# NilanEkanayake/TiTok-Video

Measured on AMD Instinct MI355X. Metric: video clips/sec encode+decode (whole node), higher is better.
Workload: dtype bf16

## Files before the change

### titok_video_amd/csrc/ttv_api.hip

```cpp
#include <stdarg.h>
#include <stdio.h>
#include <stdlib.h>
#include <string.h>

#include "ttv_common.h"
#include "ttv_kernels.h"

static thread_local char g_err[512] = "";

void ttv_set_error(const char* fmt, ...) {
  va_list ap;
  va_start(ap, fmt);
  vsnprintf(g_err, sizeof(g_err), fmt, ap);
  va_end(ap);
}

int g_ttv_prof_class = 0;
bool ttv_sw_enc_latent_last() { static const bool v = ttv_env_flag("TTV_ENC_LATENT_LAST", true); return v; }
bool ttv_enc_latent_rows_only(const ttv_tower_dims* d, const ttv_batch* b) {
  return ttv_sw_enc_latent_last() && !(g_ttv_debug & TTV_DBG_ENC_ALL_ROWS) && d->kind == TTV_ENCODER && b->latent_rows && b->sum_tokens > 0 &&
         b->sum_tokens < b->total_rows;
}
bool ttv_sw_keel_f32sum() { static const bool v = ttv_env_flag("TTV_KEEL_F32SUM", false); return v; }
bool ttv_sw_fused_patch() { static const bool v = ttv_env_flag("TTV_FUSED_PATCH", true); return v; }
// ... 527 lines not shown
  return ttvk_mlp_fused(ao, ldao, attn_post_gain, attn_alpha, x, ldx, mlp_packed, inner, y, ldy, ffd_post_gain, ffd_alpha, eps, M,
                        next ? &nx : nullptr, (hipStream_t)stream);
}

int ttv_fill_const_rows(void* x, int dtype, int ld, const int32_t* rows_map, int rows, int width, const float* mask_token,
                        const float* gain, float eps, void* stream) {
  TTV_CHECK_ARG(rows == 0 || (x && rows_map && mask_token && gain), "fill_const_rows: null buffer");
  return ttvk_fill_const_rows(x, dtype, ld, rows_map, rows, width, mask_token, gain, eps, (hipStream_t)stream);
}

int ttv_decoder_embed(const void* codes, int token_size, const void* w, const void* bias, const float* mask_token, const float* gain,
                      void* x, int dtype, int ld, const int32_t* rows_map, int rows, int width, float eps, void* stream) {
  TTV_CHECK_ARG(rows == 0 || (codes && w && bias && mask_token && gain && x && rows_map), "decoder_embed: null buffer");
  return ttvk_dec_embed(codes, token_size, w, bias, mask_token, gain, x, dtype, ld, rows_map, rows, width, eps, (hipStream_t)stream);
}

int ttv_attention(const void* qkvg, int ld, void* out, int ldo, const int32_t* cu_seqlens, const int32_t* qblocks, int n_qblocks,
                  int q_heads, int kv_heads, int head_dim, int flags, int dtype, void* stream) {
  TTV_CHECK_ARG(n_qblocks == 0 || (qkvg && out && cu_seqlens && qblocks), "attention: null buffer");
  return ttvk_attention(qkvg, ld, out, ldo, cu_seqlens, qblocks, n_qblocks, q_heads, kv_heads, head_dim, flags, dtype, (hipStream_t)stream);
}
int ttv_attention64(const void* qkvg, int ld, void* out, int ldo, const int32_t* cu_seqlens, const int32_t* items, int n_items, int q_heads,
                    int kv_heads, int head_dim, int flags, int dtype, void* stream) {
  TTV_CHECK_ARG(dtype == TTV_BF16 && head_dim == 64, "attention64: bf16, head_dim 64 only");
  return ttvk_attention64(qkvg, ld, out, ldo, cu_seqlens, items, n_items, q_heads, kv_heads, flags, (hipStream_t)stream);
}

int ttv_rmsnorm_mx(const void* in, int in_dtype, int ld_in, void* out, int out_dtype, int ld_out, const float* gain, int rows, int width,
                   float eps, float* next_rstd, void* mx_q, void* mx_s, void* stream) {
  TTV_CHECK_ARG(rows >= 0 && (rows == 0 || (in && out && gain)), "rmsnorm_mx: null buffer");
  TTV_CHECK_ARG(!mx_q == !mx_s, "rmsnorm_mx: the image needs both its element and its scale buffer");
  return ttvk_rmsnorm(in, in_dtype, ld_in, nullptr, out, out_dtype, ld_out, nullptr, gain, rows, width, eps, (hipStream_t)stream, next_rstd, mx_q, mx_s);
}

int ttv_attention_mxout(const void* qkvg, int ld, void* out_q, void* out_mx, int ld_mx, const int32_t* cu_seqlens, const int32_t* qblocks,
                        int n_qblocks, int q_heads, int kv_heads, void* stream) {
  TTV_CHECK_ARG(n_qblocks >= 0 && (n_qblocks == 0 || (qkvg && out_q && out_mx && cu_seqlens && qblocks)), "attention_mxout: null buffer");
  return ttvk_attention_mxout(qkvg, ld, out_q, out_mx, ld_mx, cu_seqlens, qblocks, n_qblocks, q_heads, kv_heads, (hipStream_t)stream);
}

int ttv_linear_fp8_mx_geglu_q(const void* xq, int ldx, const void* x_mx, const float* x_row_scale, const void* wq, int ldw, const void* w_mx,
                              const float* w_row_scale, void* hq, void* hq_mx, int M, int N, int K, void* stream) {
  TTV_CHECK_ARG(M == 0 || (xq && wq && x_mx && w_mx && hq && hq_mx), "linear_fp8_mx_geglu_q: null buffer");
  GemmArgs a = gemm_args(TTV_BF16, xq, ldx, wq, ldw, M, N, K, hq, N);
  a.yq = hq; a.yq_mx = hq_mx;
  return ttvk_gemm_fp8(EPI_GEGLU, a, x_row_scale, w_row_scale, (hipStream_t)stream, x_mx, w_mx);
}

int ttv_row_rstd(const void* x, int dtype, int ldx, float* rstd, int rows, int width, float eps, void* stream) {
  TTV_CHECK_ARG(rows >= 0 && (rows == 0 || (x && rstd)), "row_rstd: null buffer");
  TTV_CHECK_ARG(ldx >= width, "row_rstd: leading dim smaller than the width");
  return ttvk_row_rstd(x, dtype, ldx, rstd, rows, width, eps, (hipStream_t)stream);
}

int ttv_linear_rowscale(const void* x, int ldx, const void* w, int ldw, const float* row_scale, int epilogue, const float* rope_cs, int d_model,
                        int gqa_dim, void* y, int ldy, int M, int N, int K, int dtype, void* stream) {
  TTV_CHECK_ARG(M == 0 || (x && w && y), "linear_rowscale: null buffer");
  TTV_CHECK_ARG(epilogue >= 0 && epilogue <= 2, "linear_rowscale: epilogue 0 (store), 1 (qkv + rotary) or 2 (GEGLU)");
  GemmArgs a = gemm_args(dtype, x, ldx, w, ldw, M, N, K, y, ldy);
  if (epilogue == 1) {
    TTV_CHECK_ARG(rope_cs && N == 2 * d_model + 2 * gqa_dim && K == d_model, "linear_rowscale: qkv epilogue needs rope_cs, N = 2 d_model + 2 gqa_dim and K = d_model");
    a = gemm_rope_qk(a, rope_cs, d_model, gqa_dim);
  }
  a.row_scale = row_scale;
  return ttvk_gemm(epilogue == 0 ? EPI_STORE : epilogue == 1 ? EPI_QKV_ROPE : EPI_GEGLU, a, (hipStream_t)stream);
}

int ttv_patch_gather(const void* const* clips, const int32_t* clip_desc, int clip0, int n_clips, int patch_t, int patch_h, int patch_w,
                     int channels, void* patches, int ld, int dtype, int max_patches_per_clip, void* stream) {
  TTV_CHECK_ARG(n_clips == 0 || (clips && clip_desc && patches), "patch_gather: null buffer");
  return ttvk_patch_copy(false, (void* const*)clips, clip_desc, clip0, n_clips, patch_t, patch_h, patch_w, channels, patches, ld, dtype, max_patches_per_clip, (hipStream_t)stream);
}

int ttv_patch_embed_norm(const void* const* clips, const int32_t* clip_desc, const int32_t* patch_rows, const int32_t* row_seq, int n_clips,
                         int patch_t, int patch_h, int patch_w, int channels, const void* w, int ldw, const void* bias, const float* mask_token,
                         const float* gain, float eps, void* x, int ldx, int rows, int width, int dtype, void* stream) {
  TTV_CHECK_ARG(rows == 0 || (clips && clip_desc && patch_rows && row_seq && w && bias && mask_token && gain && x), "patch_embed_norm: null buffer");
  const int pd = channels * patch_t * patch_h * patch_w;
  if (!ttvk_patch_embed_norm_supported(dtype, width, pd, patch_w)) {
    ttv_set_error("patch_embed_norm: only bf16, width 256, patch_w 8 and a patch vector that is a multiple of 64");
    return TTV_ERR_UNSUPPORTED;
  }
  return ttvk_patch_embed_norm((void* const*)clips, 0, n_clips, clip_desc, patch_rows, row_seq, patch_t, patch_h, patch_w, pd, w, ldw, bias,
                               mask_token, gain, eps, x, ldx, rows, (hipStream_t)stream);
}

int ttv_patch_scatter(const void* patches, int ld, const int32_t* clip_desc, int clip0, int n_clips, int patch_t, int patch_h, int patch_w,
                      int channels, void* const* clips, int dtype, int max_patches_per_clip, void* stream) {
  TTV_CHECK_ARG(n_clips == 0 || (clips && clip_desc && patches), "patch_scatter: null buffer");
  return ttvk_patch_copy(true, clips, clip_desc, clip0, n_clips, patch_t, patch_h, patch_w, channels, (void*)patches, ld, dtype, max_patches_per_clip, (hipStream_t)stream);
}

int64_t ttv_tower_workspace_bytes(const ttv_tower_dims* dims, const ttv_batch* batch) {
  if (check_dims(dims, batch) != TTV_OK) return -1;
  return carve(dims, batch, nullptr).total;
}

int ttv_encoder_forward(const ttv_tower_dims* d, const ttv_tower_weights* w, const ttv_batch* b, const void* const* clips,
                        const ttv_fsq_params* fsq, float* z, void* codes, int32_t* indices, float* bounded, void* workspace,
                        int64_t workspace_bytes, void* stream) {
  TTV_TRY(check_dims(d, b));
  TTV_CHECK_ARG(d->kind == TTV_ENCODER, "encoder_forward: dims.kind is not TTV_ENCODER");
  TTV_CHECK_ARG(w && w->layers && clips && workspace, "encoder_forward: null argument");
  TTV_CHECK_ARG(fsq || z, "encoder_forward: neither fsq nor z requested");
  TTV_CHECK_ARG(!fsq || (codes && indices), "encoder_forward: fsq needs codes and indices buffers");
  hipStream_t s = (hipStream_t)stream;
  TowerWs ws = carve(d, b, (char*)workspace);
  TTV_CHECK_ARG(ws.total <= workspace_bytes, "encoder_forward: workspace too small (%lld < %lld)", (long long)workspace_bytes, (long long)ws.total);
  const int dm = d->width, dt = d->dtype, P = b->sum_patches, pd = patch_dim(d);

  static const bool embed_env = ttv_env_flag("TTV_PATCH_EMBED_FUSED", true);
  if (embed_env && !(g_ttv_debug & TTV_DBG_PATCH_EMBED_UNFUSED) && fused_patch_ok(d, b, dt) && w->proj_in_b && w->mask_token &&
      ttvk_patch_embed_norm_supported(dt, dm, pd, d->patch_w)) {
    TTV_TRY(ttvk_patch_embed_norm((void* const*)clips, 0, b->n_clips, b->clip_desc, b->patch_rows, b->row_seq, d->patch_t, d->patch_h, d->patch_w,
                                  pd, w->proj_in_w, pd, w->proj_in_b, w->mask_token, w->ln_pre_p, d->eps, ws.x, dm, P, s));
  } else {
    const bool gather = fused_patch_ok(d, b, dt) && pd != 256;
    if (!gather) TTV_TRY(patch_copy_all(false, (void* const*)clips, d, b, ws.pa, dt, s));
    GemmArgs a = gemm_args(dt, ws.pa, pd, w->proj_in_w, pd, P, dm, pd, ws.pb, dm);
    a.bias = w->proj_in_b; a.add_scalar = w->mask_token;
    a.split3 = (dt == TTV_F32 && w->f32_split3) ? 1 : 0;
    if (gather) {
      a.gather = 1; a.clips = (void* const*)clips; a.n_clips = b->n_clips; a.clip_desc = b->clip_desc; a.patch_rows = b->patch_rows;
      a.row_seq = b->row_seq; a.patch_t = d->patch_t; a.patch_h = d->patch_h; a.patch_w = d->patch_w;
    }
    TTV_TRY(ttvk_gemm(EPI_STORE, a, s));
    TTV_TRY(ttvk_rmsnorm(ws.pb, dt, dm, nullptr, ws.x, dt, dm, b->patch_rows, w->ln_pre_p, P, dm, d->eps, s));
  }
  TTV_TRY(ttvk_fill_const_rows(ws.x, dt, dm, b->latent_rows, b->sum_tokens, dm, w->mask_token, w->ln_pre_t, d->eps, s));

  TTV_TRY(run_layers(d, w, b, ws, s));

  TTV_TRY(ttvk_enc_tail(ws.x, dt, dm, b->latent_rows, b->sum_tokens, dm, w->ln_post, d->eps, w->proj_out_w, w->proj_out_b, d->token_size, fsq, z, codes, indices, bounded, s));
  return TTV_OK;
}

int64_t ttv_dec_l0_const_bytes(const ttv_tower_dims* d, int patch_rows) {
  if (!d || patch_rows <= 0 || d->dtype != TTV_BF16 || d->width != 256 || d->head_dim != 64 || d->kv_heads <= 0) {
    ttv_set_error("dec_l0_const_bytes: bf16 decoders of width 256 and head_dim 64 only");
    return -1;
  }
  if (patch_rows % 128) {
    ttv_set_error("dec_l0_const_bytes: patch_rows must be a multiple of 128");
    return -1;
  }
  const int64_t nq = 2 * (int64_t)d->width + 2 * (int64_t)d->kv_heads * d->head_dim;
  return align256(patch_rows * nq * 2) + align256(ttvk_attention_swp_state_floats(patch_rows, d->q_heads) * 4 + 4) + align256((int64_t)patch_rows * d->width * 2);
}

int ttv_dec_l0_const_build(const ttv_tower_dims* d, const ttv_tower_weights* w, const int32_t* iota, const float* rope_cs, const int32_t* rope_ids,
                           const float* rope_base, int patch_rows, void* block, int64_t block_bytes, int64_t* state_offset, int64_t* flag_offset,
                           void* stream) {
  TTV_CHECK_ARG(d && w && w->layers && iota && rope_cs && block && patch_rows > 0, "dec_l0_const_build: null argument");
  const int64_t need = ttv_dec_l0_const_bytes(d, patch_rows);
  if (need < 0) return TTV_ERR_UNSUPPORTED;
  TTV_CHECK_ARG(d->kind == TTV_DECODER && need <= block_bytes && (uintptr_t)block % 256 == 0, "dec_l0_const_build: not a decoder, or block too small / unaligned");
  const ttv_layer_weights& lw = w->layers[0];
  if (!lw.to_qkv_pn || !lw.qkv_q_prescaled) {
    ttv_set_error("dec_l0_const_build: layer 0 needs the folded, q-pre-scaled to_qkv weight");
    return TTV_ERR_UNSUPPORTED;
  }
  hipStream_t s = (hipStream_t)stream;
  const int dm = d->width, g = d->kv_heads * d->head_dim, nq = 2 * dm + 2 * g, dt = d->dtype;
  char* const rows = (char*)block;
  const int64_t state_floats = ttvk_attention_swp_state_floats(patch_rows, d->q_heads);
  float* const state = (float*)(rows + align256((int64_t)patch_rows * nq * 2));
  char* const x = (char*)state + align256(state_floats * 4 + 4);
  if (state_offset) *state_offset = (char*)state - rows;
  if (flag_offset) *flag_offset = (char*)(state + state_floats) - rows;
  TTV_TRY(ttvk_fill_const_rows(x, dt, dm, iota, patch_rows, dm, w->mask_token, w->ln_pre_p, d->eps, s));
  GemmArgs a = gemm_rope_qk(gemm_args(dt, x, dm, lw.to_qkv_pn, dm, patch_rows, nq, dm, rows, nq), rope_cs, dm, g);
  a.prenorm = 1; a.eps = d->eps;
  a.rope_ids = rope_ids; a.rope_base = rope_ids ? rope_base : nullptr;
  TTV_TRY(ttvk_gemm(EPI_QKV_ROPE, a, s));
  if (hipMemsetAsync(state + state_floats, 0, 4, s) != hipSuccess) {
    ttv_set_error("dec_l0_const_build: hipMemsetAsync failed");
    return TTV_ERR_LAUNCH;
  }
  return ttvk_attention_swp_dump(rows, nq, patch_rows, d->q_heads, d->kv_heads, state, s);
}

int ttv_decoder_forward(const ttv_tower_dims* d, const ttv_tower_weights* w, const ttv_batch* b, const void* codes,
                        void* const* clips_out, void* workspace, int64_t workspace_bytes, void* stream) {
  return ttv_decoder_forward_const(d, w, b, codes, clips_out, workspace, workspace_bytes, nullptr, stream);
}

int ttv_decoder_forward_const(const ttv_tower_dims* d, const ttv_tower_weights* w, const ttv_batch* b, const void* codes,
                              void* const* clips_out, void* workspace, int64_t workspace_bytes, const ttv_dec_l0_const* l0, void* stream) {
  TTV_TRY(check_dims(d, b));
  TTV_CHECK_ARG(d->kind == TTV_DECODER, "decoder_forward: dims.kind is not TTV_DECODER");
  TTV_CHECK_ARG(w && w->layers && codes && clips_out && workspace, "decoder_forward: null argument");
  hipStream_t s = (hipStream_t)stream;
  TowerWs ws = carve(d, b, (char*)workspace);
  TTV_CHECK_ARG(ws.total <= workspace_bytes, "decoder_forward: workspace too small (%lld < %lld)", (long long)workspace_bytes, (long long)ws.total);
  const int dm = d->width, dt = d->dtype, P = b->sum_patches, pd = patch_dim(d);

  TTV_TRY(ttvk_dec_embed(codes, d->token_size, w->proj_in_w, w->proj_in_b, w->mask_token, w->ln_pre_t, ws.x, dt, dm, b->latent_rows, b->sum_tokens, dm, d->eps, s));
  TTV_TRY(ttvk_fill_const_rows(ws.x, dt, dm, b->patch_rows, P, dm, w->mask_token, w->ln_pre_p, d->eps, s));

  TTV_TRY(run_layers(d, w, b, ws, s, l0));

  GemmArgs a = gemm_args(dt, nullptr, dm, w->proj_out_w, dm, P, pd, dm, ws.pa, pd);
  a.split3 = (dt == TTV_F32 && w->f32_split3) ? 1 : 0;
  a.bias = w->proj_out_b;
  if (dt == TTV_BF16 && dm == 256 && w->proj_out_pn && pd % 8 == 0) {
    a.x = ws.x; a.x_rows = b->patch_rows; a.w = w->proj_out_pn; a.prenorm = 1; a.eps = d->eps;
  } else {
    TTV_TRY(ttvk_rmsnorm(ws.x, dt, dm, b->patch_rows, ws.pb, dt, dm, nullptr, w->ln_post, P, dm, d->eps, s));
    a.x = ws.pb;
  }
  if (fused_patch_ok(d, b, dt) && dm == 256) {
    a.clips = clips_out; a.n_clips = b->n_clips; a.clip_desc = b->clip_desc; a.patch_rows = b->patch_rows; a.row_seq = b->row_seq;
// ... 197 lines not shown
```

### titok_video_amd/csrc/ttv_kernels.h

```cpp
#pragma once
#include <hip/hip_runtime.h>
#include <stdint.h>

#include "../../include/titok_hip.h"

int ttvk_rmsnorm(const void* in, int in_dtype, int ld_in, const int* src_rows, void* out, int out_dtype, int ld_out,
                 const int* dst_rows, const float* gain, int rows, int d, float eps, hipStream_t s, float* next_rstd = nullptr,
                 void* mx_q = nullptr, void* mx_s = nullptr,
                 int split_image = 0);
int ttvk_row_rstd(const void* in, int dtype, int ld_in, float* rstd, int rows, int d, float eps, hipStream_t s);
int ttvk_copy_rows(const void* src, int64_t ld_src_bytes, const int* src_rows, void* dst, int64_t ld_dst_bytes, const int* dst_rows, int rows,
                   int row_bytes, hipStream_t s);
int ttvk_fill_const_rows(void* x, int dtype, int ld, const int* rows_map, int rows, int d, const float* mask_token,
                         const float* gain, float eps, hipStream_t s);
int ttvk_dec_embed(const void* codes, int C, const void* w, const void* bias, const float* mask_token, const float* gain,
                   void* x, int dtype, int ld, const int* rows_map, int rows, int d, float eps, hipStream_t s);
int ttvk_fsq_forward(const ttv_fsq_params* p, const void* z, int z_dtype, int rows, void* codes, int codes_dtype, int* indices,
                     float* bounded, hipStream_t s);
int ttvk_fsq_indices_to_codes(const ttv_fsq_params* p, const int* indices, int rows, void* codes, int codes_dtype, hipStream_t s);
int ttvk_enc_tail(const void* x, int dtype, int ld, const int* rows_map, int rows, int d, const float* gain, float eps,
                  const void* w, const void* bias, int C, const ttv_fsq_params* fsq, float* z_out, void* codes, int* indices,
                  float* bounded, hipStream_t s);
int ttvk_patch_copy(bool scatter, void* const* clips, const int* clip_desc, int clip0, int n_clips, int pt, int ph, int pw,
                    int C, void* patches, int ld, int dtype, int max_patches, hipStream_t s);
int ttvk_rope_apply(void* x, int dtype, int ld, int rows, int heads, const float* cs, hipStream_t s);
int ttvk_histogram(const int* idx, int n, int64_t* counts, int size, hipStream_t s);
int ttvk_quant_rows_fp8(const void* in, int in_dtype, int ld_in, const float* gain, float eps, void* out, int ld_out, float* scales, int rows,
                        int d, hipStream_t s);

int ttvk_split3_pack(const float* w, int ldw, void* out, int ldo, int rows, int K, hipStream_t s);
int64_t ttvk_mx_scale_ld(int d);
int ttvk_quant_mx_fp8(const void* in, int in_dtype, int ld_in, void* out, int ld_out, void* mx, float* row_scales, int rows, int d, hipStream_t s);

int ttvk_clip_from_u8(const void* frames, long long n_pix, void* clip, int dtype, hipStream_t s);

int ttvk_clip_resample_u8(void* const* src, void* const* dst, const int32_t* geom, int n_clips, int dtype, hipStream_t s);

enum GemmEpilogue {
  EPI_STORE = 0,
  EPI_QKV_ROPE,
  EPI_GEGLU,
  EPI_RESID_T,
  EPI_RESID_F32,
  EPI_RESID_NORM,
  EPI_STORE_PATCH,
  EPI_BIAS_PLAIN,
  EPI_BIAS_GELU,
  EPI_BIAS_RESID_F32R,
};

struct GemmArgs {
  const void* x; int ldx;
  const void* w; int ldw;
  int M, N, K;
  void* y; int ldy;
  const void* bias;
  const float* add_scalar;
  const void* resid; int ldr;
  float alpha;
  const float* rope_cs;
  const int* rope_ids; const float* rope_base;
  int rope_q_end, rope_k_begin, rope_k_end;
  int dtype;
  const float* norm_gain;
  float* sum_f32; int ld_sum;
  void* y2; int ldy2; const float* norm_gain2;
  void* yq; void* yq_mx;
  int split3;
  int x_image, y_image;
  int prenorm;
  const float* row_scale;
  const int* x_rows;
  float eps;
  int gather;
  void* const* clips;
  int n_clips;
  const int* clip_desc;
  const int* patch_rows;
  const int* row_seq;
  int patch_t, patch_h, patch_w;
  int resid_rows;
  int tile_run, tile_period;
  int panel_lo;
};
struct ClipPtrs { void* p[TTV_MAX_CLIPS_PER_LAUNCH]; };
int ttvk_gemm(GemmEpilogue epi, const GemmArgs& a, hipStream_t s);
int ttvk_gemm_fp8(GemmEpilogue epi, const GemmArgs& a, const float* x_scale, const float* w_scale, hipStream_t s, const void* x_mx = nullptr,
                  const void* w_mx = nullptr);
bool ttvk_gemm_supports_resid_norm(int dtype, int N, int K);
bool ttvk_gemm_qkv_tiles_supported(int d_model, int gqa_dim, int ldw);

bool ttvk_patch_embed_norm_supported(int dtype, int width, int patch_dim, int patch_w);
int ttvk_patch_embed_norm(void* const* clips, int clip0, int n_clips, const int* clip_desc, const int* patch_rows, const int* row_seq,
                          int patch_t, int patch_h, int patch_w, int patch_dim, const void* w, int ldw, const void* bias,
                          const float* mask_token, const float* gain, float eps, void* x, int ldx, int M, hipStream_t s);

int ttvk_attention(const void* qkvg, int ld, void* out, int ldo, const int* cu_seqlens, const int* qblocks, int n_qblocks,
                   int q_heads, int kv_heads, int head_dim, int flags, int dtype, hipStream_t s, float* lse_out = nullptr,
                   void* out_raw = nullptr);

bool ttvk_attention_takes_swp(int flags);
int ttvk_attention_swp(const void* qkvg, int ld, void* out, int ldo, const int* cu_seqlens, const int* qblocks, int n_qblocks,
                       int q_heads, int kv_heads, int gate_mul, hipStream_t s, const void* rows2 = nullptr, int kwin = 0,
                       const float* state = nullptr);
int64_t ttvk_attention_swp_state_floats(int n_rows, int q_heads);
int ttvk_attention_swp_dump(const void* rows, int ld, int n_rows, int q_heads, int kv_heads, float* state, hipStream_t s);
int ttvk_attention_mxout(const void* qkvg, int ld, void* out_q, void* out_mx, int ld_mx, const int* cu_seqlens, const int* qblocks,
                         int n_qblocks, int q_heads, int kv_heads, hipStream_t s);

int ttvk_attention64(const void* qkvg, int ld, void* out, int ldo, const int* cu_seqlens, const int* items, int n_items, int q_heads,
                     int kv_heads, int flags, hipStream_t s);

int ttvk_vq_norms(const void* cb, int dtype, int ld, int N, int C, float* cnorm, hipStream_t s);
int64_t ttvk_vq_workspace_bytes(int rows);
int ttvk_vq_l2_argmin(const void* z, int dtype, int ldz, const void* cb, int ldc, const float* cnorm, int rows, int N, int C, int* indices,
                      float* best_dist, void* workspace, int64_t workspace_bytes, hipStream_t s);
int ttvk_vq_lookup(const void* cb, int dtype, int ldc, const int* indices, int rows, int C, void* codes, int ldo, hipStream_t s);
int ttvk_vq_lookup_bwd(const void* dcodes, int dtype, int ld, const int* indices, int rows, int C, float* dcb, int ldc, hipStream_t s);

int64_t ttvk_vq_train_workspace_bytes(int rows, int N);
int ttvk_vq_commit_forward(const void* z, int dtype, int ldz, const void* cb, int ldc, const int* idx, int rows, int N, int C, float* loss,
                           void* workspace, int64_t workspace_bytes, hipStream_t s);
int ttvk_vq_commit_backward(const void* g, int ldg, const void* z, int ldz, const void* e, int lde, int dtype, int rows, int C, double scale,
                            void* dz, int ldd, hipStream_t s);
int ttvk_vq_ema_stats(const void* z, int dtype, int ldz, const int* idx, int rows, int N, int C, const float* cluster_size, float dead_threshold,
                      uint64_t seed, const int64_t* ema_step, int rank, int world_size, float* stats, void* workspace, int64_t workspace_bytes,
                      hipStream_t s);
int ttvk_vq_ema_update(const float* stats, float* cluster_size, float* embed_avg, float* codebook, void* copy, int copy_dtype, float* cnorm,
                       int64_t* ema_step, int N, int C, float decay, float one_minus_decay, float eps, float dead_threshold, void* workspace,
                       int64_t workspace_bytes, hipStream_t s);

bool ttvk_mlp_fused_supported(int dtype, int width, int inner);
struct MlpNextQkv {
  void* qkv; int ld;
  const float* rope_cs;
  int rows;
  int rope_q_end, rope_k_begin, rope_k_end;
};
int64_t ttvk_mlp_pack_bytes(int inner, int next_qkv_rows);
int ttvk_mlp_pack(const void* w12_folded, const void* w3, const void* wo, const void* next_qkv_folded, int next_qkv_rows, int inner,
                  void* packed, hipStream_t s);
int ttvk_mlp_fused(const void* ao, int ldao, const float* front_gain, float front_alpha, const void* x, int ldx, const void* packed,
                   int inner, void* y, int ldy, const float* post_gain, float alpha, float eps, int M, const MlpNextQkv* nq, hipStream_t s);

int ttvk_l1_loss(void* const* recon, void* const* target, void* const* grad, const int* sizes, int n_clips, int total_clips, int dtype,
                 float* loss, hipStream_t s);
int ttvk_sq_err(void* const* recon, void* const* target, const int* sizes, int n_clips, int dtype, int clamp, double* acc2, hipStream_t s);
int ttvk_rmsnorm_bwd_chain(const void* x, int ldx, const void* dy, int lddy, const float* gain1, float* dgain1, float* dx, int lddx,
                           const void* y, int y_dt, int ldy, const float* gain2, float* dgain2, float out_scale, void* cast_out, int ldc, int rows,
                           int d, float eps, int dt, hipStream_t s);
int ttvk_rmsnorm_bwd(const void* x, int x_dt, int ldx, const int* xr, const void* dy, int dy_dt, int lddy, const int* dyr,
                     const float* gain, void* dx, int dx_dt, int lddx, const int* dxr, int acc, float* dgain, int rows, int d, float eps,
                     hipStream_t s);
int ttvk_colsum(const void* a, int dt, int lda, const int* rows_map, int rows, int n, float* out, hipStream_t s);
int ttvk_sumall(const void* a, int dt, int lda, const int* rows_map, int rows, int n, const float* colw, float scale, float* out, hipStream_t s);
int ttvk_gate_fwd(const void* a, int lda, const void* gate, int ldg, void* ag, int ldo, int rows, int d, int dt, hipStream_t s);
int ttvk_gate_bwd(const void* dag, int ldd, const void* a, int lda, const void* gate, int ldg, void* da, int ldda, void* dgate, int lddg,
                  int rows, int d, int dt, float* delta, hipStream_t s);
int ttvk_geglu_fwd(const void* u, int ldu, void* h, int ldh, int rows, int I, int dt, hipStream_t s);
int ttvk_geglu_bwd(const void* u, int ldu, const void* dh, int lddh, void* du, int lddu, int rows, int I, int dt, hipStream_t s);
int ttvk_scale_cast(const float* a, float alpha, float* b, void* c, int dt, long n, hipStream_t s);
int ttvk_to_f32(const void* a, int dt, float* b, long n, int accumulate, hipStream_t s);
int ttvk_fsq_bwd(const ttv_fsq_params* fp, const float* z, const void* dcodes, int dt, float* dz, int rows, hipStream_t s);
#define TTV_WGRAD_BATCH 6
struct WgradBatch {
  int n = 0;
  int64_t used_bytes = 0;
  struct Entry { const float* part; float* dw; int splits, lddw, N, K, tiles_n, tiles; } e[TTV_WGRAD_BATCH];
};
int ttvk_wgrad(const void* dy, int lddy, const void* x, int ldx, float* dw, int lddw, int L, int N, int K, int dt, float* part,
               int64_t part_bytes, hipStream_t s, WgradBatch* batch = nullptr);
int ttvk_wgrad_flush(WgradBatch* batch, hipStream_t s);
int64_t ttvk_wgrad_ws_bytes(int L, int N, int K);
int ttvk_outer_small(const void* a, int a_dt, int lda, int C, const void* b, int b_dt, int ldb, const int* b_rows, float* dw, int lddw,
                     int transpose_out, int rows, int d, hipStream_t s);
int ttvk_expand_small(const void* a, int a_dt, int lda, int C, const void* w, int w_dt, int ldw, int w_cf, void* out, int o_dt, int ldo,
                      int rows, int d, hipStream_t s);
int ttvk_reduce_small(const void* a, int a_dt, int lda, const int* a_rows, const void* w, int w_dt, int ldw, int C, float* out, int ldo,
// ... 100 lines not shown
```

### titok_video_amd/csrc/ttv_patch_embed.hip

```cpp
#include "ttv_common.h"
#include "ttv_kernels.h"

#define PE_TT 128
#define PE_F 256
#define PE_BK 64
#define PE_STAGES 3
#define PE_STAGE_U4 ((PE_F + PE_TT) * 8)

struct PatchEmbedDev {
  ClipPtrs clips;
  const int* clip_desc; const int* patch_rows; const int* row_seq;
  const bf16_t* w; const bf16_t* bias; const float* mask_token; const float* gain;
  bf16_t* x;
  int ldw, ldx, M, K, clip0, pt_shift, ph_shift;
  float eps;
};

__global__ __launch_bounds__(512, 1) void k_patch_embed256(PatchEmbedDev p) {
  __shared__ __attribute__((aligned(16))) uint4 lds[PE_STAGES][PE_STAGE_U4];
  const int tid = threadIdx.x, lane = tid & 63;
  const int wave = __builtin_amdgcn_readfirstlane(tid >> 6);
  const int wf = wave & 1, wt = wave >> 1;
  const int tbase = blockIdx.x * PE_TT;

  const int lr = lane >> 3, lp = lane & 7;
  uint32_t woff[4];
#pragma unroll
  for (int i = 0; i < 4; ++i) {
    const int row = wave * 32 + i * 8 + lr;
    woff[i] = ((uint32_t)row * (uint32_t)p.ldw + (uint32_t)((lp ^ ((row >> 1) & 7)) * 8)) * 2u;
  }
  const bf16_t* gbase[2];
  int gthw[2], ghw[2], gw_[2], gch[2];
#pragma unroll
  for (int i = 0; i < 2; ++i) {
    const int row = wave * 16 + i * 8 + lr;
    int t = tbase + row;
    t = t < p.M ? t : p.M - 1;
    const int ci = p.row_seq[p.patch_rows[t]];
    const int* ds = p.clip_desc + (size_t)ci * 8;
    const int Tn = ds[0], H = ds[1], W = ds[2], gh = ds[4], gw = ds[5], pl = t - ds[6];
    const int gwi = pl % gw, r = pl / gw, ghi = r % gh, gti = r / gh;
    gthw[i] = Tn * H * W; ghw[i] = H * W; gw_[i] = W;
    gch[i] = lp ^ ((row >> 1) & 7);
    gbase[i] = reinterpret_cast<const bf16_t*>(p.clips.p[ci - p.clip0]) + ((size_t)((gti << p.pt_shift) * H + (ghi << p.ph_shift)) * W + gwi * 8);
  }
  const uint32_t lds0 = (uint32_t)(uintptr_t)(__attribute__((address_space(3))) void*)&lds[0][0];
  constexpr uint32_t STAGEB = PE_STAGE_U4 * 16;
#define PE_DMA_W(voff_, base_, dst_)                                                                             \
  do {                                                                                                           \
    unsigned keep__;                                                                                             \
    asm volatile("s_mov_b32 %0, m0\n\ts_mov_b32 m0, %3\n\ts_nop 0\n\tglobal_load_lds_dwordx4 %1, %2\n\ts_mov_b32 m0, %0" \
                 : "=&s"(keep__) : "v"(voff_), "s"(base_), "s"(dst_) : "memory");                                 \
  } while (0)
#define PE_DMA_X(ptr_, dst_)                                                                                     \
  do {                                                                                                           \
    unsigned keep__;                                                                                             \
    asm volatile("s_mov_b32 %0, m0\n\ts_mov_b32 m0, %2\n\ts_nop 0\n\tglobal_load_lds_dwordx4 %1, off\n\ts_mov_b32 m0, %0" \
                 : "=&s"(keep__) : "v"(ptr_), "s"(dst_) : "memory");                                              \
  } while (0)
#define PE_STAGE(kt_, st_)                                                                                       \
  do {                                                                                                           \
    const bf16_t* wb__ = p.w + (size_t)(kt_) * PE_BK;                                                            \
    const uint32_t dw__ = lds0 + (st_) * STAGEB + wave * 4096;                                                   \
    const uint32_t dx__ = lds0 + (st_) * STAGEB + PE_F * 128 + wave * 2048;                                      \
    _Pragma("unroll") for (int i__ = 0; i__ < 4; ++i__) PE_DMA_W(woff[i__], wb__, dw__ + i__ * 1024);            \
    _Pragma("unroll") for (int i__ = 0; i__ < 2; ++i__) {                                                        \
      const int sg__ = (kt_) * 8 + gch[i__];                                                                     \
      const int c__ = sg__ >> (p.pt_shift + p.ph_shift), ipt__ = (sg__ >> p.ph_shift) & ((1 << p.pt_shift) - 1); \
      const int iph__ = sg__ & ((1 << p.ph_shift) - 1);                                                          \
      const bf16_t* src__ = gbase[i__] + ((size_t)c__ * gthw[i__] + (size_t)ipt__ * ghw[i__] + (size_t)iph__ * gw_[i__]); \
      PE_DMA_X(src__, dx__ + i__ * 1024);                                                                        \
    }                                                                                                            \
  } while (0)

  f32x4 acc[8][2];
#pragma unroll
  for (int i = 0; i < 8; ++i)
#pragma unroll
    for (int j = 0; j < 2; ++j) acc[i][j] = (f32x4){0.f, 0.f, 0.f, 0.f};

  const int l15 = lane & 15, kq = lane >> 4;
  const int nk = p.K / PE_BK;
  const char* const ldsb = reinterpret_cast<const char*>(&lds[0][0]);
  const uint32_t fo0 = (uint32_t)(l15 * 128 + (((0 + kq) ^ ((l15 >> 1) & 7)) << 4));
  const uint32_t fo1 = (uint32_t)(l15 * 128 + (((4 + kq) ^ ((l15 >> 1) & 7)) << 4));
  const uint32_t a_base = (uint32_t)(wf * 128 * 128), b_base = (uint32_t)(PE_F * 128 + wt * 32 * 128);

  asm volatile("s_waitcnt vmcnt(0)" ::: "memory");
  PE_STAGE(0, 0);
  if (nk > 1) PE_STAGE(1, 1);
  int st = 0;
  for (int kt = 0; kt < nk; ++kt) {
    if (kt + 1 < nk) asm volatile("s_waitcnt vmcnt(6)" ::: "memory");
    else asm volatile("s_waitcnt vmcnt(0)" ::: "memory");
    __syncthreads();
    if (kt + 2 < nk) {
      const int st2 = st + 2 >= PE_STAGES ? st + 2 - PE_STAGES : st + 2;
      PE_STAGE(kt + 2, st2);
    }
    const char* const sb = ldsb + (size_t)st * STAGEB;
#pragma unroll
    for (int ks = 0; ks < 2; ++ks) {
      const uint32_t fo = ks ? fo1 : fo0;
      bf16x8 a[8], b[2];
#pragma unroll
      for (int i = 0; i < 8; ++i) a[i] = *reinterpret_cast<const bf16x8*>(sb + a_base + fo + i * 2048);
#pragma unroll
      for (int j = 0; j < 2; ++j) b[j] = *reinterpret_cast<const bf16x8*>(sb + b_base + fo + j * 2048);
#pragma unroll
      for (int i = 0; i < 8; ++i)
#pragma unroll
        for (int j = 0; j < 2; ++j) acc[i][j] = __builtin_amdgcn_mfma_f32_16x16x32_bf16(a[i], b[j], acc[i][j], 0, 0, 0);
    }
    st = st + 1 == PE_STAGES ? 0 : st + 1;
  }
#undef PE_STAGE
#undef PE_DMA_W
#undef PE_DMA_X

  const float sc = round_to<bf16_t>(p.mask_token[0]);
  float* const gx = reinterpret_cast<float*>(&lds[st][0]);
  float grp[8][2];
#pragma unroll
  for (int i = 0; i < 8; ++i) {
    const int f = wf * 128 + i * 16 + kq * 4;
    const f32x4 bv = Vec4<bf16_t>::load(p.bias + f);
#pragma unroll
    for (int j = 0; j < 2; ++j) {
      acc[i][j] += bv;
#pragma unroll
      for (int e = 0; e < 4; ++e)
        acc[i][j][e] = round_to<bf16_t>(round_to<bf16_t>(acc[i][j][e]) + sc);
      const f32x4 y = acc[i][j];
      grp[i][j] = fmaf(y[3], y[3], fmaf(y[2], y[2], fmaf(y[0], y[0], y[1] * y[1])));
      gx[(wf * PE_TT + wt * 32 + j * 16 + l15) * 33 + i * 4 + kq] = grp[i][j];
    }
  }
  __syncthreads();
#pragma unroll
  for (int j = 0; j < 2; ++j) {
    const int tl = wt * 32 + j * 16 + l15;
    const int t = tbase + tl;
    float s1[8];
#pragma unroll
    for (int i = 0; i < 8; ++i) s1[i] = grp[i][j] + gx[((wf ^ 1) * PE_TT + tl) * 33 + i * 4 + kq];
    const float t0 = s1[0] + s1[4], t1 = s1[1] + s1[5], t2 = s1[2] + s1[6], t3 = s1[3] + s1[7];
    float tot = (t0 + t2) + (t1 + t3);
    tot = pair32_sum(tot);
    {
      const unsigned u = __float_as_uint(tot);
      const auto a = __builtin_amdgcn_permlane16_swap(u, u, false, false);
      const unsigned a0 = a[0], a1 = a[1];
      tot = __uint_as_float(a0) + __uint_as_float(a1);
    }
    const float rstd = 1.0f / sqrtf(tot / 256.0f + p.eps);
    if (t < p.M) {
      bf16_t* const q = p.x + (size_t)p.patch_rows[t] * p.ldx;
#pragma unroll
      for (int i = 0; i < 8; ++i) {
        const int f = wf * 128 + i * 16 + kq * 4;
        const f32x4 g = *reinterpret_cast<const f32x4*>(p.gain + f);
        const f32x4 o = {acc[i][j][0] * rstd * g[0], acc[i][j][1] * rstd * g[1], acc[i][j][2] * rstd * g[2], acc[i][j][3] * rstd * g[3]};
        Vec4<bf16_t>::store(q + f, o);
      }
    }
  }
}

bool ttvk_patch_embed_norm_supported(int dtype, int width, int patch_dim, int patch_w) {
  return dtype == TTV_BF16 && width == PE_F && patch_dim % PE_BK == 0 && patch_dim >= PE_BK && patch_w == 8;
}

int ttvk_patch_embed_norm(void* const* clips, int clip0, int n_clips, const int* clip_desc, const int* patch_rows, const int* row_seq,
                          int patch_t, int patch_h, int patch_w, int patch_dim, const void* w, int ldw, const void* bias,
                          const float* mask_token, const float* gain, float eps, void* x, int ldx, int M, hipStream_t s) {
  if (M == 0) return TTV_OK;
  auto lg2 = [](int v) { int sh = 0; while ((1 << sh) < v) ++sh; return (1 << sh) == v ? sh : -1; };
  TTV_CHECK_ARG(patch_w == 8 && lg2(patch_t) >= 0 && lg2(patch_h) >= 0 && patch_dim % PE_BK == 0 && patch_dim >= PE_BK &&
                    patch_dim % (patch_t * patch_h * patch_w) == 0,
                "patch_embed_norm: patch_w == 8, power-of-two patch_t / patch_h and a patch vector that is a multiple of 64");
  TTV_CHECK_ARG(n_clips > 0 && n_clips <= TTV_MAX_CLIPS_PER_LAUNCH, "patch_embed_norm: 1 .. %d clips per call", TTV_MAX_CLIPS_PER_LAUNCH);
  TTV_CHECK_ARG(ldw >= patch_dim && ldw % 8 == 0 && ldx >= PE_F && ldx % 4 == 0 && (uint64_t)PE_F * (uint64_t)ldw * 2u < (1ull << 32),
                "patch_embed_norm: leading dims must hold a row and keep its alignment");
  TTV_CHECK_ARG((uintptr_t)w % 16 == 0 && (uintptr_t)x % 8 == 0 && (uintptr_t)bias % 8 == 0 && (uintptr_t)gain % 16 == 0,
                "patch_embed_norm: pointers must keep their vector alignment");
  PatchEmbedDev d;
  for (int i = 0; i < n_clips; ++i) {
    TTV_CHECK_ARG(clips[i] && (uintptr_t)clips[i] % 16 == 0, "patch_embed_norm: clip %d is null or not 16-byte aligned", i);
    d.clips.p[i] = clips[i];
  }
  for (int i = n_clips; i < TTV_MAX_CLIPS_PER_LAUNCH; ++i) d.clips.p[i] = nullptr;
  d.clip_desc = clip_desc; d.patch_rows = patch_rows; d.row_seq = row_seq;
  d.w = (const bf16_t*)w; d.bias = (const bf16_t*)bias; d.mask_token = mask_token; d.gain = gain; d.x = (bf16_t*)x;
  d.ldw = ldw; d.ldx = ldx; d.M = M; d.K = patch_dim; d.clip0 = clip0; d.pt_shift = lg2(patch_t); d.ph_shift = lg2(patch_h);
  d.eps = eps;
  TtvProfScope prof(TTV_KC_GEMM_STORE, s);
  hipLaunchKernelGGL(k_patch_embed256, dim3(ttv_cdiv(M, PE_TT)), dim3(512), 0, s, d);
  TTV_CHECK_LAUNCH("patch_embed256");
  return TTV_OK;
}
```

Before: 32130.

## Fold latent-row fill into patch embed kernel and stage output through LDS

The separate fill_const_rows launch is removed. The patch-embed kernel now gets extra blocks that write the constant normalized mask-token rows for latent positions. The main tile path preloads bias, gain and row indices before the K loop and splits W and X staging into separate macros. The epilogue now writes results to LDS and emits coalesced 16-byte row stores instead of scattered 8-byte stores. It also adds optional compile-time probes (timestamps and knockouts of W, X or LDS reads), and it tightens the ldx and x alignment requirements to 16 bytes.

```diff
diff --git a/titok_video_amd/csrc/ttv_api.hip b/titok_video_amd/csrc/ttv_api.hip
--- a/titok_video_amd/csrc/ttv_api.hip
+++ b/titok_video_amd/csrc/ttv_api.hip
@@ -633,7 +633,7 @@
     return TTV_ERR_UNSUPPORTED;
   }
   return ttvk_patch_embed_norm((void* const*)clips, 0, n_clips, clip_desc, patch_rows, row_seq, patch_t, patch_h, patch_w, pd, w, ldw, bias,
-                               mask_token, gain, eps, x, ldx, rows, (hipStream_t)stream);
+                               mask_token, gain, eps, x, ldx, rows, nullptr, 0, nullptr, (hipStream_t)stream);
 }
 
 int ttv_patch_scatter(const void* patches, int ld, const int32_t* clip_desc, int clip0, int n_clips, int patch_t, int patch_h, int patch_w,
@@ -664,7 +664,8 @@
   if (embed_env && !(g_ttv_debug & TTV_DBG_PATCH_EMBED_UNFUSED) && fused_patch_ok(d, b, dt) && w->proj_in_b && w->mask_token &&
       ttvk_patch_embed_norm_supported(dt, dm, pd, d->patch_w)) {
     TTV_TRY(ttvk_patch_embed_norm((void* const*)clips, 0, b->n_clips, b->clip_desc, b->patch_rows, b->row_seq, d->patch_t, d->patch_h, d->patch_w,
-                                  pd, w->proj_in_w, pd, w->proj_in_b, w->mask_token, w->ln_pre_p, d->eps, ws.x, dm, P, s));
+                                  pd, w->proj_in_w, pd, w->proj_in_b, w->mask_token, w->ln_pre_p, d->eps, ws.x, dm, P, b->latent_rows,
+                                  b->sum_tokens, w->ln_pre_t, s));
   } else {
     const bool gather = fused_patch_ok(d, b, dt) && pd != 256;
     if (!gather) TTV_TRY(patch_copy_all(false, (void* const*)clips, d, b, ws.pa, dt, s));
@@ -677,8 +678,8 @@
     }
     TTV_TRY(ttvk_gemm(EPI_STORE, a, s));
     TTV_TRY(ttvk_rmsnorm(ws.pb, dt, dm, nullptr, ws.x, dt, dm, b->patch_rows, w->ln_pre_p, P, dm, d->eps, s));
-  }
-  TTV_TRY(ttvk_fill_const_rows(ws.x, dt, dm, b->latent_rows, b->sum_tokens, dm, w->mask_token, w->ln_pre_t, d->eps, s));
+    TTV_TRY(ttvk_fill_const_rows(ws.x, dt, dm, b->latent_rows, b->sum_tokens, dm, w->mask_token, w->ln_pre_t, d->eps, s));
+  }
 
   TTV_TRY(run_layers(d, w, b, ws, s));
 
diff --git a/titok_video_amd/csrc/ttv_kernels.h b/titok_video_amd/csrc/ttv_kernels.h
--- a/titok_video_amd/csrc/ttv_kernels.h
+++ b/titok_video_amd/csrc/ttv_kernels.h
@@ -93,7 +93,8 @@
 bool ttvk_patch_embed_norm_supported(int dtype, int width, int patch_dim, int patch_w);
 int ttvk_patch_embed_norm(void* const* clips, int clip0, int n_clips, const int* clip_desc, const int* patch_rows, const int* row_seq,
                           int patch_t, int patch_h, int patch_w, int patch_dim, const void* w, int ldw, const void* bias,
-                          const float* mask_token, const float* gain, float eps, void* x, int ldx, int M, hipStream_t s);
+                          const float* mask_token, const float* gain, float eps, void* x, int ldx, int M, const int* latent_rows,
+                          int n_latent, const float* latent_gain, hipStream_t s);
 
 int ttvk_attention(const void* qkvg, int ld, void* out, int ldo, const int* cu_seqlens, const int* qblocks, int n_qblocks,
                    int q_heads, int kv_heads, int head_dim, int flags, int dtype, hipStream_t s, float* lse_out = nullptr,
diff --git a/titok_video_amd/csrc/ttv_patch_embed.hip b/titok_video_amd/csrc/ttv_patch_embed.hip
--- a/titok_video_amd/csrc/ttv_patch_embed.hip
+++ b/titok_video_amd/csrc/ttv_patch_embed.hip
@@ -6,22 +6,69 @@
 #define PE_BK 64
 #define PE_STAGES 3
 #define PE_STAGE_U4 ((PE_F + PE_TT) * 8)
+#ifdef PE_KO_W
+#define PE_W_PIECES 0
+#else
+#define PE_W_PIECES 4
+#endif
+#ifdef PE_KO_X
+#define PE_X_PIECES 0
+#else
+#define PE_X_PIECES 2
+#endif
 
 struct PatchEmbedDev {
   ClipPtrs clips;
-  const int* clip_desc; const int* patch_rows; const int* row_seq;
-  const bf16_t* w; const bf16_t* bias; const float* mask_token; const float* gain;
+  const int* clip_desc; const int* patch_rows; const int* row_seq; const int* latent_rows;
+  const bf16_t* w; const bf16_t* bias; const float* mask_token; const float* gain; const float* latent_gain;
   bf16_t* x;
-  int ldw, ldx, M, K, clip0, pt_shift, ph_shift;
+  long long* stamps;
+  int ldw, ldx, M, K, clip0, pt_shift, ph_shift, tile_blocks, n_latent;
   float eps;
 };
+
+#ifdef PE_STAMPS
+#define PE_STAMP(var_)                                                                                           \
+  do {                                                                                                           \
+    __builtin_amdgcn_sched_barrier(0);                                                                           \
+    asm volatile("s_memtime %0\n\ts_waitcnt lgkmcnt(0)" : "=s"(var_)::"memory");                                 \
+    __builtin_amdgcn_sched_barrier(0);                                                                           \
+  } while (0)
+#else
+#define PE_STAMP(var_)
+#endif
 
 __global__ __launch_bounds__(512, 1) void k_patch_embed256(PatchEmbedDev p) {
   __shared__ __attribute__((aligned(16))) uint4 lds[PE_STAGES][PE_STAGE_U4];
   const int tid = threadIdx.x, lane = tid & 63;
   const int wave = __builtin_amdgcn_readfirstlane(tid >> 6);
+
+  if ((int)blockIdx.x >= p.tile_blocks) {
+    const float m = round_to<bf16_t>(p.mask_token[0]);
+    const float rstd = 1.0f / sqrtf(m * m + p.eps);
+    const int c = (lane & 31) * 8;
+    const f32x4 g0 = *reinterpret_cast<const f32x4*>(p.latent_gain + c), g1 = *reinterpret_cast<const f32x4*>(p.latent_gain + c + 4);
+    const bf16x8 o = {(bf16_t)(m * rstd * g0[0]), (bf16_t)(m * rstd * g0[1]), (bf16_t)(m * rstd * g0[2]), (bf16_t)(m * rstd * g0[3]),
+                      (bf16_t)(m * rstd * g1[0]), (bf16_t)(m * rstd * g1[1]), (bf16_t)(m * rstd * g1[2]), (bf16_t)(m * rstd * g1[3])};
+    const int r0 = ((int)blockIdx.x - p.tile_blocks) * PE_TT + wave * 16 + (lane >> 5);
+    int row[8];
+#pragma unroll
+    for (int q = 0; q < 8; ++q) row[q] = p.latent_rows[r0 + 2 * q < p.n_latent ? r0 + 2 * q : p.n_latent - 1];
+#pragma unroll
+    for (int q = 0; q < 8; ++q)
+      if (r0 + 2 * q < p.n_latent) *reinterpret_cast<bf16x8*>(p.x + (size_t)row[q] * p.ldx + c) = o;
+    return;
+  }
+#ifdef PE_STAMPS
+  unsigned long long st_entry = 0, st_loop = 0, st_a = 0, st_b = 0, st_staged = 0, st_issued = 0, st_exit = 0, st_wait = 0, st_mfma = 0, st_wait0 = 0;
+  unsigned long long rt_entry = 0, rt_exit = 0;
+  PE_STAMP(st_entry);
+  asm volatile("s_memrealtime %0\n\ts_waitcnt lgkmcnt(0)" : "=s"(rt_entry)::"memory");
+#endif
   const int wf = wave & 1, wt = wave >> 1;
   const int tbase = blockIdx.x * PE_TT;
+  const int l15 = lane & 15, kq = lane >> 4;
+  const int nk = p.K / PE_BK;
 
   const int lr = lane >> 3, lp = lane & 7;
   uint32_t woff[4];
@@ -29,6 +76,47 @@
   for (int i = 0; i < 4; ++i) {
     const int row = wave * 32 + i * 8 + lr;
     woff[i] = ((uint32_t)row * (uint32_t)p.ldw + (uint32_t)((lp ^ ((row >> 1) & 7)) * 8)) * 2u;
+  }
+  const uint32_t lds0 = (uint32_t)(uintptr_t)(__attribute__((address_space(3))) void*)&lds[0][0];
+  constexpr uint32_t STAGEB = PE_STAGE_U4 * 16;
+#define PE_DMA_W(voff_, base_, dst_)                                                                             \
+  do {                                                                                                           \
+    unsigned keep__;                                                                                             \
+    asm volatile("s_mov_b32 %0, m0\n\ts_mov_b32 m0, %3\n\ts_nop 0\n\tglobal_load_lds_dwordx4 %1, %2\n\ts_mov_b32 m0, %0" \
+                 : "=&s"(keep__) : "v"(voff_), "s"(base_), "s"(dst_) : "memory");                                 \
+  } while (0)
+#define PE_DMA_X(ptr_, dst_)                                                                                     \
+  do {                                                                                                           \
+    unsigned keep__;                                                                                             \
+    asm volatile("s_mov_b32 %0, m0\n\ts_mov_b32 m0, %2\n\ts_nop 0\n\tglobal_load_lds_dwordx4 %1, off\n\ts_mov_b32 m0, %0" \
+                 : "=&s"(keep__) : "v"(ptr_), "s"(dst_) : "memory");                                              \
+  } while (0)
+#define PE_STAGE_W(kt_, st_)                                                                                     \
+  do {                                                                                                           \
+    const bf16_t* wb__ = p.w + (size_t)(kt_) * PE_BK;                                                            \
+    const uint32_t dw__ = lds0 + (st_) * STAGEB + wave * 4096;                                                   \
+    _Pragma("unroll") for (int i__ = 0; i__ < PE_W_PIECES; ++i__) PE_DMA_W(woff[i__], wb__, dw__ + i__ * 1024);  \
+  } while (0)
+#define PE_STAGE_X(kt_, st_)                                                                                     \
+  do {                                                                                                           \
+    const uint32_t dx__ = lds0 + (st_) * STAGEB + PE_F * 128 + wave * 2048;                                      \
+    _Pragma("unroll") for (int i__ = 0; i__ < PE_X_PIECES; ++i__) {                                              \
+      const int sg__ = (kt_) * 8 + gch[i__];                                                                     \
+      const int c__ = sg__ >> (p.pt_shift + p.ph_shift), ipt__ = (sg__ >> p.ph_shift) & ((1 << p.pt_shift) - 1); \
+      const int iph__ = sg__ & ((1 << p.ph_shift) - 1);                                                          \
+      const bf16_t* src__ = gbase[i__] + ((size_t)c__ * gthw[i__] + (size_t)ipt__ * ghw[i__] + (size_t)iph__ * gw_[i__]); \
+      PE_DMA_X(src__, dx__ + i__ * 1024);                                                                        \
+    }                                                                                                            \
+  } while (0)
+
+  const float mask0 = p.mask_token[0];
+  bf16x4 braw[8];
+  f32x4 gv[8];
+#pragma unroll
+  for (int i = 0; i < 8; ++i) {
+    const int f = wf * 128 + i * 16 + kq * 4;
+    braw[i] = *reinterpret_cast<const bf16x4*>(p.bias + f);
+    gv[i] = *reinterpret_cast<const f32x4*>(p.gain + f);
   }
   const bf16_t* gbase[2];
   int gthw[2], ghw[2], gw_[2], gch[2];
@@ -45,34 +133,20 @@
     gch[i] = lp ^ ((row >> 1) & 7);
     gbase[i] = reinterpret_cast<const bf16_t*>(p.clips.p[ci - p.clip0]) + ((size_t)((gti << p.pt_shift) * H + (ghi << p.ph_shift)) * W + gwi * 8);
   }
-  const uint32_t lds0 = (uint32_t)(uintptr_t)(__attribute__((address_space(3))) void*)&lds[0][0];
-  constexpr uint32_t STAGEB = PE_STAGE_U4 * 16;
-#define PE_DMA_W(voff_, base_, dst_)                                                                             \
-  do {                                                                                                           \
-    unsigned keep__;                                                                                             \
-    asm volatile("s_mov_b32 %0, m0\n\ts_mov_b32 m0, %3\n\ts_nop 0\n\tglobal_load_lds_dwordx4 %1, %2\n\ts_mov_b32 m0, %0" \
-                 : "=&s"(keep__) : "v"(voff_), "s"(base_), "s"(dst_) : "memory");                                 \
-  } while (0)
-#define PE_DMA_X(ptr_, dst_)                                                                                     \
-  do {                                                                                                           \
-    unsigned keep__;                                                                                             \
-    asm volatile("s_mov_b32 %0, m0\n\ts_mov_b32 m0, %2\n\ts_nop 0\n\tglobal_load_lds_dwordx4 %1, off\n\ts_mov_b32 m0, %0" \
-                 : "=&s"(keep__) : "v"(ptr_), "s"(dst_) : "memory");                                              \
-  } while (0)
-#define PE_STAGE(kt_, st_)                                                                                       \
-  do {                                                                                                           \
-    const bf16_t* wb__ = p.w + (size_t)(kt_) * PE_BK;                                                            \
-    const uint32_t dw__ = lds0 + (st_) * STAGEB + wave * 4096;                                                   \
-    const uint32_t dx__ = lds0 + (st_) * STAGEB + PE_F * 128 + wave * 2048;                                      \
-    _Pragma("unroll") for (int i__ = 0; i__ < 4; ++i__) PE_DMA_W(woff[i__], wb__, dw__ + i__ * 1024);            \
-    _Pragma("unroll") for (int i__ = 0; i__ < 2; ++i__) {                                                        \
-      const int sg__ = (kt_) * 8 + gch[i__];                                                                     \
-      const int c__ = sg__ >> (p.pt_shift + p.ph_shift), ipt__ = (sg__ >> p.ph_shift) & ((1 << p.pt_shift) - 1); \
-      const int iph__ = sg__ & ((1 << p.ph_shift) - 1);                                                          \
-      const bf16_t* src__ = gbase[i__] + ((size_t)c__ * gthw[i__] + (size_t)ipt__ * ghw[i__] + (size_t)iph__ * gw_[i__]); \
-      PE_DMA_X(src__, dx__ + i__ * 1024);                                                                        \
-    }                                                                                                            \
-  } while (0)
+  int my_row = -1;
+  if (lane < 16 && tbase + wave * 16 + lane < p.M) my_row = p.patch_rows[tbase + wave * 16 + lane];
+  __builtin_amdgcn_sched_barrier(0);
+  asm volatile("s_waitcnt vmcnt(0)" ::: "memory");
+  float sc = round_to<bf16_t>(mask0);
+  asm volatile("" : "+v"(sc), "+v"(my_row));
+#pragma unroll
+  for (int i = 0; i < 8; ++i) asm volatile("" : "+v"(braw[i]), "+v"(gv[i]));
+#pragma unroll
+  for (int i = 0; i < 2; ++i) asm volatile("" : "+v"(gbase[i]), "+v"(gthw[i]), "+v"(ghw[i]), "+v"(gw_[i]));
+  __builtin_amdgcn_sched_barrier(0);
+  PE_STAGE_W(0, 0);
+  PE_STAGE_X(0, 0);
+  if (nk > 1) { PE_STAGE_W(1, 1); PE_STAGE_X(1, 1); }
 
   f32x4 acc[8][2];
 #pragma unroll
@@ -80,52 +154,62 @@
 #pragma unroll
     for (int j = 0; j < 2; ++j) acc[i][j] = (f32x4){0.f, 0.f, 0.f, 0.f};
 
-  const int l15 = lane & 15, kq = lane >> 4;
-  const int nk = p.K / PE_BK;
-  const char* const ldsb = reinterpret_cast<const char*>(&lds[0][0]);
+  char* const ldsb = reinterpret_cast<char*>(&lds[0][0]);
   const uint32_t fo0 = (uint32_t)(l15 * 128 + (((0 + kq) ^ ((l15 >> 1) & 7)) << 4));
   const uint32_t fo1 = (uint32_t)(l15 * 128 + (((4 + kq) ^ ((l15 >> 1) & 7)) << 4));
   const uint32_t a_base = (uint32_t)(wf * 128 * 128), b_base = (uint32_t)(PE_F * 128 + wt * 32 * 128);
-
-  asm volatile("s_waitcnt vmcnt(0)" ::: "memory");
-  PE_STAGE(0, 0);
-  if (nk > 1) PE_STAGE(1, 1);
+  PE_STAMP(st_loop);
+#ifdef PE_STAMPS
+  st_a = st_loop;
+#endif
   int st = 0;
   for (int kt = 0; kt < nk; ++kt) {
-    if (kt + 1 < nk) asm volatile("s_waitcnt vmcnt(6)" ::: "memory");
-    else asm volatile("s_waitcnt vmcnt(0)" ::: "memory");
+    if (kt + 1 >= nk) asm volatile("s_waitcnt vmcnt(0)" ::: "memory");
+    else asm volatile("s_waitcnt vmcnt(%0)" ::"n"(PE_W_PIECES + PE_X_PIECES) : "memory");
     __syncthreads();
+    PE_STAMP(st_b);
     if (kt + 2 < nk) {
       const int st2 = st + 2 >= PE_STAGES ? st + 2 - PE_STAGES : st + 2;
-      PE_STAGE(kt + 2, st2);
+      PE_STAGE_W(kt + 2, st2);
+      PE_STAGE_X(kt + 2, st2);
     }
     const char* const sb = ldsb + (size_t)st * STAGEB;
 #pragma unroll
     for (int ks = 0; ks < 2; ++ks) {
       const uint32_t fo = ks ? fo1 : fo0;
       bf16x8 a[8], b[2];
+#ifdef PE_KO_LDS
+#pragma unroll
+      for (int i = 0; i < 8; ++i) a[i] = (bf16x8){(bf16_t)(float)(lane + i + kt), 0, 0, 0, 0, 0, 0, 0};
+#pragma unroll
+      for (int j = 0; j < 2; ++j) b[j] = (bf16x8){(bf16_t)(float)(lane + j + ks), 0, 0, 0, 0, 0, 0, 0};
+      (void)sb; (void)fo;
+#else
 #pragma unroll
       for (int i = 0; i < 8; ++i) a[i] = *reinterpret_cast<const bf16x8*>(sb + a_base + fo + i * 2048);
 #pragma unroll
       for (int j = 0; j < 2; ++j) b[j] = *reinterpret_cast<const bf16x8*>(sb + b_base + fo + j * 2048);
+#endif
 #pragma unroll
       for (int i = 0; i < 8; ++i)
 #pragma unroll
         for (int j = 0; j < 2; ++j) acc[i][j] = __builtin_amdgcn_mfma_f32_16x16x32_bf16(a[i], b[j], acc[i][j], 0, 0, 0);
     }
     st = st + 1 == PE_STAGES ? 0 : st + 1;
-  }
-#undef PE_STAGE
+#ifdef PE_STAMPS
+    { unsigned long long t__; PE_STAMP(t__); st_wait += st_b - st_a; st_mfma += t__ - st_b; if (kt == 0) st_wait0 = st_b - st_a; st_a = t__; }
+#endif
+  }
+#undef PE_STAGE_W
+#undef PE_STAGE_X
 #undef PE_DMA_W
 #undef PE_DMA_X
 
-  const float sc = round_to<bf16_t>(p.mask_token[0]);
-  float* const gx = reinterpret_cast<float*>(&lds[st][0]);
+  float* const gx = reinterpret_cast<float*>(ldsb + (size_t)st * STAGEB);
   float grp[8][2];
 #pragma unroll
   for (int i = 0; i < 8; ++i) {
-    const int f = wf * 128 + i * 16 + kq * 4;
-    const f32x4 bv = Vec4<bf16_t>::load(p.bias + f);
+    const f32x4 bv = {(float)braw[i][0], (float)braw[i][1], (float)braw[i][2], (float)braw[i][3]};
 #pragma unroll
     for (int j = 0; j < 2; ++j) {
       acc[i][j] += bv;
@@ -138,10 +222,12 @@
     }
   }
   __syncthreads();
+  const int st1 = st + 1 == PE_STAGES ? 0 : st + 1, st2 = st1 + 1 == PE_STAGES ? 0 : st1 + 1;
+  char* const tile_w = ldsb + (size_t)(wt < 2 ? st1 : st2) * STAGEB;
+  const char* const tile_r = ldsb + (size_t)(wave < 4 ? st1 : st2) * STAGEB;
 #pragma unroll
   for (int j = 0; j < 2; ++j) {
     const int tl = wt * 32 + j * 16 + l15;
-    const int t = tbase + tl;
     float s1[8];
 #pragma unroll
     for (int i = 0; i < 8; ++i) s1[i] = grp[i][j] + gx[((wf ^ 1) * PE_TT + tl) * 33 + i * 4 + kq];
@@ -155,17 +241,49 @@
       tot = __uint_as_float(a0) + __uint_as_float(a1);
     }
     const float rstd = 1.0f / sqrtf(tot / 256.0f + p.eps);
-    if (t < p.M) {
-      bf16_t* const q = p.x + (size_t)p.patch_rows[t] * p.ldx;
-#pragma unroll
-      for (int i = 0; i < 8; ++i) {
-        const int f = wf * 128 + i * 16 + kq * 4;
-        const f32x4 g = *reinterpret_cast<const f32x4*>(p.gain + f);
-        const f32x4 o = {acc[i][j][0] * rstd * g[0], acc[i][j][1] * rstd * g[1], acc[i][j][2] * rstd * g[2], acc[i][j][3] * rstd * g[3]};
-        Vec4<bf16_t>::store(q + f, o);
-      }
-    }
-  }
+#pragma unroll
+    for (int i = 0; i < 8; ++i) {
+      const f32x4 g = gv[i];
+      const bf16x4 o = {(bf16_t)(acc[i][j][0] * rstd * g[0]), (bf16_t)(acc[i][j][1] * rstd * g[1]), (bf16_t)(acc[i][j][2] * rstd * g[2]),
+                        (bf16_t)(acc[i][j][3] * rstd * g[3])};
+      const int chunk = wf * 16 + i * 2 + (kq >> 1);
+      *reinterpret_cast<bf16x4*>(tile_w + (tl & 63) * 512 + ((chunk ^ l15) << 4) + (kq & 1) * 8) = o;
+    }
+  }
+  __syncthreads();
+  PE_STAMP(st_staged);
+  {
+    const int half = lane >> 5, ch = lane & 31;
+    int row[8];
+    bf16x8 v[8];
+#pragma unroll
+    for (int q = 0; q < 8; ++q) {
+      const int rl = 2 * q + half;
+      row[q] = __shfl(my_row, rl);
+      v[q] = *reinterpret_cast<const bf16x8*>(tile_r + ((wave & 3) * 16 + rl) * 512 + ((ch ^ rl) << 4));
+    }
+    __builtin_amdgcn_sched_barrier(0);
+#pragma unroll
+    for (int q = 0; q < 8; ++q)
+      if (row[q] >= 0) *reinterpret_cast<bf16x8*>(p.x + (size_t)row[q] * p.ldx + ch * 8) = v[q];
+  }
+#ifdef PE_STAMPS
+  PE_STAMP(st_issued);
+  asm volatile("s_waitcnt vmcnt(0)" ::: "memory");
+  PE_STAMP(st_exit);
+  asm volatile("s_memrealtime %0\n\ts_waitcnt lgkmcnt(0)" : "=s"(rt_exit)::"memory");
+  if (p.stamps && blockIdx.x % 8 == 0 && lane == 0) {
+    long long* dst = p.stamps + ((size_t)(blockIdx.x / 8) * 8 + wave) * 8;
+    dst[0] = (long long)(st_loop - st_entry);
+    dst[1] = (long long)st_wait;
+    dst[2] = (long long)st_mfma;
+    dst[3] = (long long)(st_issued - st_a);
+    dst[4] = (long long)(st_exit - st_entry);
+    dst[5] = (long long)st_wait0;
+    dst[6] = (long long)(st_staged - st_a);
+    dst[7] = (long long)(rt_exit - rt_entry);
+  }
+#endif
 }
 
 bool ttvk_patch_embed_norm_supported(int dtype, int width, int patch_dim, int patch_w) {
@@ -174,29 +292,33 @@
 
 int ttvk_patch_embed_norm(void* const* clips, int clip0, int n_clips, const int* clip_desc, const int* patch_rows, const int* row_seq,
                           int patch_t, int patch_h, int patch_w, int patch_dim, const void* w, int ldw, const void* bias,
-                          const float* mask_token, const float* gain, float eps, void* x, int ldx, int M, hipStream_t s) {
-  if (M == 0) return TTV_OK;
+                          const float* mask_token, const float* gain, float eps, void* x, int ldx, int M, const int* latent_rows,
+                          int n_latent, const float* latent_gain, hipStream_t s) {
+  if (M == 0 && n_latent == 0) return TTV_OK;
   auto lg2 = [](int v) { int sh = 0; while ((1 << sh) < v) ++sh; return (1 << sh) == v ? sh : -1; };
   TTV_CHECK_ARG(patch_w == 8 && lg2(patch_t) >= 0 && lg2(patch_h) >= 0 && patch_dim % PE_BK == 0 && patch_dim >= PE_BK &&
                     patch_dim % (patch_t * patch_h * patch_w) == 0,
                 "patch_embed_norm: patch_w == 8, power-of-two patch_t / patch_h and a patch vector that is a multiple of 64");
-  TTV_CHECK_ARG(n_clips > 0 && n_clips <= TTV_MAX_CLIPS_PER_LAUNCH, "patch_embed_norm: 1 .. %d clips per call", TTV_MAX_CLIPS_PER_LAUNCH);
-  TTV_CHECK_ARG(ldw >= patch_dim && ldw % 8 == 0 && ldx >= PE_F && ldx % 4 == 0 && (uint64_t)PE_F * (uint64_t)ldw * 2u < (1ull << 32),
+  TTV_CHECK_ARG(M == 0 || (n_clips > 0 && n_clips <= TTV_MAX_CLIPS_PER_LAUNCH), "patch_embed_norm: 1 .. %d clips per call", TTV_MAX_CLIPS_PER_LAUNCH);
+  TTV_CHECK_ARG(ldw >= patch_dim && ldw % 8 == 0 && ldx >= PE_F && ldx % 8 == 0 && (uint64_t)PE_F * (uint64_t)ldw * 2u < (1ull << 32),
                 "patch_embed_norm: leading dims must hold a row and keep its alignment");
-  TTV_CHECK_ARG((uintptr_t)w % 16 == 0 && (uintptr_t)x % 8 == 0 && (uintptr_t)bias % 8 == 0 && (uintptr_t)gain % 16 == 0,
+  TTV_CHECK_ARG((uintptr_t)w % 16 == 0 && (uintptr_t)x % 16 == 0 && (uintptr_t)bias % 8 == 0 && (uintptr_t)gain % 16 == 0,
                 "patch_embed_norm: pointers must keep their vector alignment");
+  TTV_CHECK_ARG(n_latent == 0 || (latent_rows && latent_gain && (uintptr_t)latent_gain % 16 == 0), "patch_embed_norm: latent rows without their map or gain");
   PatchEmbedDev d;
-  for (int i = 0; i < n_clips; ++i) {
+  for (int i = 0; i < (M ? n_clips : 0); ++i) {
     TTV_CHECK_ARG(clips[i] && (uintptr_t)clips[i] % 16 == 0, "patch_embed_norm: clip %d is null or not 16-byte aligned", i);
     d.clips.p[i] = clips[i];
   }
-  for (int i = n_clips; i < TTV_MAX_CLIPS_PER_LAUNCH; ++i) d.clips.p[i] = nullptr;
-  d.clip_desc = clip_desc; d.patch_rows = patch_rows; d.row_seq = row_seq;
-  d.w = (const bf16_t*)w; d.bias = (const bf16_t*)bias; d.mask_token = mask_token; d.gain = gain; d.x = (bf16_t*)x;
+  for (int i = (M ? n_clips : 0); i < TTV_MAX_CLIPS_PER_LAUNCH; ++i) d.clips.p[i] = nullptr;
+  d.clip_desc = clip_desc; d.patch_rows = patch_rows; d.row_seq = row_seq; d.latent_rows = latent_rows;
+  d.w = (const bf16_t*)w; d.bias = (const bf16_t*)bias; d.mask_token = mask_token; d.gain = gain; d.latent_gain = latent_gain; d.x = (bf16_t*)x;
+  d.stamps = g_ttv_stamps;
   d.ldw = ldw; d.ldx = ldx; d.M = M; d.K = patch_dim; d.clip0 = clip0; d.pt_shift = lg2(patch_t); d.ph_shift = lg2(patch_h);
+  d.tile_blocks = ttv_cdiv(M, PE_TT); d.n_latent = n_latent;
   d.eps = eps;
   TtvProfScope prof(TTV_KC_GEMM_STORE, s);
-  hipLaunchKernelGGL(k_patch_embed256, dim3(ttv_cdiv(M, PE_TT)), dim3(512), 0, s, d);
+  hipLaunchKernelGGL(k_patch_embed256, dim3(d.tile_blocks + ttv_cdiv(n_latent, PE_TT)), dim3(512), 0, s, d);
   TTV_CHECK_LAUNCH("patch_embed256");
   return TTV_OK;
 }
```

Result: no change. 32340, median of 4 (+0.6%).
